# cts198859/deeprl_signal_control

Measured on NVIDIA H100. Metric: agent-env-steps/sec, higher is better.
Workload: dtype f32 (sim, LSTM cell, loss, optimizer) + bf16 tensor-core operands with f32 accumulation (learner GEMMs)

## Files before the change

deeprl_signal_control_b200/_lib.py:

```python
from __future__ import annotations

import ctypes as C
import os
import subprocess

_HERE = os.path.dirname(os.path.abspath(__file__))
CSRC = os.path.join(_HERE, "csrc")
LIB_PATH = os.environ.get("TSC_LIB", os.path.join(CSRC, "libtsc.so"))
_lib = None

SYMBOLS = ["tsc_last_error", "tsc_create", "tsc_destroy", "tsc_reset", "tsc_set_train_mode",
           "tsc_set_replica_coop_gamma", "tsc_observe", "tsc_step", "tsc_step_host", "tsc_step_host_range", "tsc_step_host_range_async", "tsc_set_record", "tsc_step_record", "tsc_get_trips", "tsc_get_counts", "tsc_get_traffic_stats",
           "tsc_dump_state", "tsc_info", "tsc_mean_live", "tsc_set_greedy_program", "tsc_greedy_actions",
           "tscl_create", "tscl_destroy", "tscl_fc_embed", "tscl_lstm_seq_fwd", "tscl_heads", "tscl_returns", "tscl_returns_g",
           "tscl_heads_loss", "tscl_lstm_seq_bwd", "tscl_fc_bwd", "tscl_fc_bwd_tc", "tscl_wgrad_tc", "tscl_clip_rmsprop",
           "tscl_pack_weights", "tscl_policy_step", "tscl_policy_step_v2", "tscl_policy_step_v2r", "tscl_policy_step_v2g", "tscl_unpack_store", "tscl_pack_wht", "tscl_lstm_seq_bwd_tc", "tscl_pack_wxt", "tscl_lstm_seq_bwd_tc_dx", "tscl_lstm_seq_bwd_tc_heads", "tscl_dx_tc", "tscl_dx_fc_bwd_tc", "tscl_host_transition", "tscl_device_transition", "tscl_device_transition_g","tscl_memcpy_async", "tscl_fc_hidden_fwd", "tscl_fc_hidden_bwd", "tscl_debug_policy_prof", "tscl_debug_bptt_prof",
           "tscl_policy_step_pi", "tscl_argmax_actions", "tscl_q_create", "tscl_q_destroy", "tscl_q_step",
           "tscl_q_explore", "tscl_q_sample", "tscl_q_td", "tscl_q_adam", "tscl_q_transition"]


def build_native(force: bool = False, verbose: bool = False) -> str:
    cmd = ["make", "-C", CSRC] + (["-B"] if force else [])
    out = subprocess.run(cmd, capture_output=True, text=True)
    if out.returncode != 0:
        raise RuntimeError("nvcc build of libtsc.so failed:\n" + out.stdout + out.stderr)
    if verbose:
        print(out.stdout + out.stderr)
    return LIB_PATH


def lib() -> C.CDLL:
    global _lib
    if _lib is None:
        if not os.path.exists(LIB_PATH):
            raise ImportError(
                "native library %s is missing: run `python -c 'import __graft_entry__ as g; g.build()'` "
                "(there is no CPU fallback)" % LIB_PATH)
        _lib = C.CDLL(LIB_PATH)
        _lib.tsc_last_error.restype = C.c_char_p
        for s in SYMBOLS:
            getattr(_lib, s)
    return _lib


def check(rc: int):
    if rc != 0:
        raise RuntimeError("libtsc: " + lib().tsc_last_error().decode())
```

deeprl_signal_control_b200/agents/learner.py:

```python
from __future__ import annotations

import ctypes as C
import os
import types
from typing import Optional, Sequence

import numpy as np
import torch

from .. import _lib
from .. import dist as _dist
from .layout import PolicyLayout


def _p(t):
    return None if t is None else C.c_void_p(t.data_ptr())


def check_population(seeds, seed, n_replicas, chunk, process_group):
    if seeds is None:
        return [int(seed)]
    seeds = [int(s) for s in seeds]
    if not seeds:
        raise ValueError("a population needs at least one seed")
# ... 127 lines not shown
        self.obs_hist = torch.zeros(T + 1, R, L.n_obs, **f32)
        self.act_hist = torch.zeros(T, R, A, dtype=torch.int32, device=self.dev)
        self.rew_hist = torch.zeros(T, R, A, **f32)
        self.val_hist = torch.zeros(T, R, A, **f32)
        self.Rs = torch.zeros(T, R, A, **f32); self.Adv = torch.zeros(T, R, A, **f32)
        self.done_pre = [0.0] * T
        self.done_post = [0.0] * T
        self.last_done = False
        self.t = 0
        self.n_forward = 0
        self._one = torch.zeros(1, **f32)
        self._upd_bufs = None
        self.kernel_launches = 0
        paths = self.paths
        self.use_tc, self.tc_v2 = paths.use_tc, paths.tc_v2
        mdim = () if self.K == 1 else (self.K,)
        self.Wp = torch.zeros(*mdim, U, ((L.dx + L.h) // 8) * 4 * L.h * 8 + 8 * L.dx * 8, dtype=torch.bfloat16,
                              device=self.dev)
        self.Wt = torch.zeros(*mdim, U, 32, L.h, 8, dtype=torch.bfloat16, device=self.dev)
        self.Wxt = torch.zeros(*mdim, U, 32, L.dx, 8, dtype=torch.bfloat16, device=self.dev)
        self.seeds_dev = torch.tensor(self.seeds, dtype=torch.int64, device=self.dev) if self.K > 1 else None
        differ = lambda *keys: any(len({h[k] for h in self.hp}) > 1 for k in keys)
        per = lambda key: torch.tensor([h[key] for h in self.hp], **f32)
        self.gamma_dev = per("gamma") if differ("gamma") else None
        self.rscale_differs = differ("reward_norm", "reward_clip")
        self.rnorm_dev, self.rclip_dev = (per("reward_norm"), per("reward_clip")) if self.rscale_differs else (None, None)
        self.dx_fused = False
        self.dx_fusable = paths.dx_fusable
        self.dx_own = paths.dx_own
        self.dx_fc_fused = paths.dx_fc_fused
        self.bwd_tc, self.fc_bwd_tc, self.wgrad_tc = paths.bwd_tc, paths.fc_bwd_tc, paths.wgrad_tc
        self.fused_heads = True
        self.heads_in_bptt = os.environ.get("TSC_BPTT_HEADS", "1") != "0"
        self._dz_all = None
        self.pack_weights()
        need = U * T * R * (L.dx + 4 * L.h + 2 * L.h) * 2
        if store_acts is None:
            free, _ = torch.cuda.mem_get_info(self.dev)
            store_acts = self.tc_v2 and need < 0.5 * free
        self.store_acts = bool(store_acts) and self.tc_v2 and (R % self.chunk == 0)
        if self.K > 1 and not self.store_acts:
            raise ValueError("a population back-propagates through the activation store, which does not fit: %.2f GB "
                             "for %d x %d replicas" % (need / 1e9, self.K, self.R_m))
        self.st_x = self.st_g = self.st_c = self.st_h = None
        if self.store_acts:
            bf = dict(dtype=torch.bfloat16, device=self.dev)
            nc, rc_ = R // self.chunk, self.chunk
            self.st_x = torch.zeros(nc, U, T, rc_, L.dx, **bf); self.st_g = torch.zeros(nc, U, T, rc_, 4 * L.h, **bf)
            self.st_c = torch.zeros(nc, U, T, rc_, L.h, **bf); self.st_h = torch.zeros(nc, U, T, rc_, L.h, **bf)
        self._acts_ok = [False] * T

    def close(self):
        if getattr(self, "_h", None) is not None:
            _lib.lib().tscl_destroy(self._h)
            self._h = None

    def __del__(self):
        try:
            self.close()
        except Exception:
            pass

    def member(self, k: int):
        if self.K == 1:
            return self
        return types.SimpleNamespace(lay=self.lay, _h=self._h, dev=self.dev, use_tc=self.use_tc, tc_v2=self.tc_v2,
# ... 188 lines not shown
        M = T * b["rc"]
        if (dh or not lean) and "dH" not in b:
            b["dH"] = torch.empty(U, M, L.h, **f32)
        if lean and dzb and "dZb" not in b:
            b["dZb"] = torch.empty(U, M, 4 * L.h, dtype=torch.bfloat16, device=self.dev)
        if lean and dxb and "dXb" not in b:
            b["dXb"] = torch.empty(U, M, L.dx, dtype=torch.bfloat16, device=self.dev)
        if not lean and "X" not in b:
            b.update(ZG=torch.empty(U, M, 4 * L.h, **f32), dX=torch.empty(U, M, L.dx, **f32),
                     X=torch.empty(U, M, L.dx, **f32), C=torch.empty(U, M, L.h, **f32), H=torch.empty(U, M, L.h, **f32),
                     Hp=torch.empty(U, M, L.h, **f32), dlog=torch.empty(U, M, L.max_na, **f32))
        return b

    def _dz_all_buf(self):
        if self._dz_all is None:
            L, nc = self.lay, self.R // self.chunk
            need = nc * L.U * self.T * self.chunk * 4 * L.h * 2
            free, _ = torch.cuda.mem_get_info(self.dev)
            if need >= 0.5 * free:
                return None
            if self._upd_bufs is not None:
                self._upd_bufs.pop("dZb", None)
            self._dz_all = torch.empty(nc, L.U, self.T * self.chunk, 4 * L.h, dtype=torch.bfloat16, device=self.dev)
        return self._dz_all

    def _bwd_heads(self, P, G, Wt, stats, r0, n_chunks, v_coef, beta, scale, dpre, dZb):
        ci, R, A = r0 // self.chunk, self.R, self.lay.A
        _lib.check(_lib.lib().tscl_lstm_seq_bwd_tc_heads(
            self._h, _p(Wt), _p(P), _p(self.st_g[ci]), _p(self.st_c[ci]), _p(self.st_h[ci]), _p(self.c_bw), _p(dpre),
            _p(self.act_hist[0, r0:]), _p(self.Rs[0, r0:]), _p(self.Adv[0, r0:]), C.c_int32(self.T),
            C.c_int64(self.chunk), C.c_int32(n_chunks), C.c_int64(R), C.c_int64(r0), C.c_int64(R * A), C.c_float(v_coef),
            C.c_float(beta), C.c_float(scale), _p(dZb), _p(stats), _p(G), self._st()))

    def backward(self, boot: Optional[torch.Tensor], lr: float, beta: float):
        assert self.t == self.T, "rollout buffer not full"
        L, R, T, U, A, lib = self.lay, self.R, self.T, self.lay.U, self.lay.A, _lib.lib()
        lrs, betas = self._per_member(lr, "lr"), self._per_member(beta, "beta")
        self._mm()
        st = self._st
        f32 = dict(dtype=torch.float32, device=self.dev)
        dpre = torch.tensor(self.done_pre, **f32)
        dpost = torch.tensor(self.done_post, **f32)
        if boot is None:
            self.boot.zero_()
        else:
            self.boot.copy_(boot)
        if self.gamma_dev is not None:
            _lib.check(lib.tscl_returns_g(self._h, _p(self.rew_hist), _p(self.val_hist), _p(self.boot), _p(dpost),
                                          _p(self.gamma_dev), C.c_int32(self.K), C.c_int32(T), C.c_int64(R), _p(self.Rs),
                                          _p(self.Adv), st()))
        else:
            _lib.check(lib.tscl_returns(self._h, _p(self.rew_hist), _p(self.val_hist), _p(self.boot), _p(dpost),
                                        C.c_float(self.gamma), C.c_int32(T), C.c_int64(R), _p(self.Rs), _p(self.Adv), st()))
        self.G.zero_()
        self.stats.zero_()
        scale = _dist.grad_scale(T, 1, self.total_replicas)
        use_store = self.store_acts and all(self._acts_ok)
        if self.K > 1 and not use_store:
            raise RuntimeError("a population update needs every step of the rollout in the activation store")
        n_obs = L.n_obs
        P, G, Wt, Wxt, stats = self.P, self.G, self.Wt, self.Wxt, self.stats
        k = 0
        lean = use_store and self.bwd_tc and self.fc_bwd_tc and self.wgrad_tc and self.fused_heads
        heads_bptt = lean and self.heads_in_bptt and not (self.dx_fused and self.dx_fusable)
        dz_all = self._dz_all_buf() if heads_bptt and self.K == 1 and R > self.chunk else None
        if dz_all is not None:
            self._bwd_heads(P, G, Wt, stats, 0, R // self.chunk, self.hp[0]["v_coef"], betas[0], scale, dpre, dz_all)
            self.kernel_launches += 1
        for r0 in range(0, R, self.chunk):
            if self.K > 1:
                k = r0 // self.R_m
                P, G, Wt, Wxt, stats = self.P[k], self.G[k], self.Wt[k], self.Wxt[k], self.stats[k]
            rc = min(self.chunk, R - r0)
            M = T * rc
            ci = r0 // self.chunk
            all_tc = lean
            fuse_dx = all_tc and self.dx_fused and self.dx_fusable
            fuse_fc = all_tc and not fuse_dx and self.dx_fc_fused
            b = self._bufs(rc, lean=all_tc, dxb=not fuse_fc, dh=not heads_bptt, dzb=dz_all is None)
            X = Cc = H = Hp = dlog = ZG = dX = dZb = dXb = dH = None
            bf16 = dict(dtype=torch.bfloat16, device=self.dev)
            if b["rc"] == rc:
                dH = b.get("dH")
                if all_tc:
                    dZb, dXb = (b["dZb"] if dz_all is None else dz_all[ci]), b.get("dXb")
                else:
                    ZG, dX, X, Cc, H, Hp, dlog = (b[k] for k in ("ZG", "dX", "X", "C", "H", "Hp", "dlog"))
            else:
                dH = torch.empty(U, M, L.h, **f32)
                if all_tc:
                    dZb = torch.empty(U, M, 4 * L.h, **bf16)
                    dXb = None if fuse_fc else torch.empty(U, M, L.dx, **bf16)
                else:
                    ZG, dX, X, Cc, H, Hp, dlog = (torch.empty(U, M, s_, **f32) for s_ in
                                                  (4 * L.h, L.dx, L.dx, L.h, L.h, L.h, L.max_na))
            obs0 = self.obs_hist[0, r0:]
            if all_tc:
                pass
            elif use_store:
                direct = self.bwd_tc
# ... 8 lines not shown
                torch.baddbmm(self.pv["bl"].unsqueeze(1), X, self.pv["wx"], out=ZG)
                _lib.check(lib.tscl_lstm_seq_fwd(self._h, _p(P), _p(ZG), _p(Cc), _p(H), _p(Hp), _p(self.c_bw),
                                                 _p(self.h_bw), None, None, _p(dpre), C.c_int32(T), C.c_int64(rc),
                                                 C.c_int64(R), C.c_int64(r0), st()))
            hb = _p(self.st_h[ci]) if use_store else None
            if heads_bptt:
                if dz_all is None:
                    self._bwd_heads(P, G, Wt, stats, r0, 1, self.hp[k]["v_coef"], betas[k], scale, dpre, dZb)
                    self.kernel_launches += 1
            else:
                _lib.check(lib.tscl_heads_loss(self._h, _p(P), None if all_tc else _p(H), _p(self.act_hist[0, r0:]),
                                               _p(self.Rs[0, r0:]), _p(self.Adv[0, r0:]), C.c_int64(M), C.c_int64(rc),
                                               C.c_int64(R * A), C.c_float(self.hp[k]["v_coef"]), C.c_float(betas[k]),
                                               C.c_float(scale),
                                               None if self.fused_heads else _p(dlog), _p(dH), _p(stats),
                                               hb if all_tc else None, _p(G) if self.fused_heads else None, st()))
                self.kernel_launches += 2
            if not self.fused_heads:
                self.gv["wo"].baddbmm_(H.transpose(1, 2), dlog)
                self.gv["bo"].add_(dlog.sum(dim=1))
            if heads_bptt:
                pass
            elif self.bwd_tc:
                gb = (_p(self.st_g[ci]), _p(self.st_c[ci])) if use_store else (None, None)
                _lib.check(lib.tscl_lstm_seq_bwd_tc_dx(self._h, _p(Wt), _p(ZG), _p(Cc), _p(dH), _p(self.c_bw),
                                                       _p(dpre), C.c_int32(T), C.c_int64(rc), C.c_int64(R), C.c_int64(r0),
                                                       *gb, _p(dZb), _p(Wxt) if fuse_dx else None,
                                                       _p(dXb) if fuse_dx else None, st()))
            else:
                _lib.check(lib.tscl_lstm_seq_bwd(self._h, _p(P), _p(ZG), _p(Cc), _p(dH), _p(self.c_bw), _p(dpre),
                                                 C.c_int32(T), C.c_int64(rc), C.c_int64(R), C.c_int64(r0), st()))
            dZ = ZG
            if self.wgrad_tc:
                if use_store:
                    _lib.check(lib.tscl_wgrad_tc(self._h, _p(dZ), _p(dZb), None, _p(self.st_x[ci]), None, _p(self.st_h[ci]),
                                                 _p(self.h_bw), _p(dpre), C.c_int32(T), C.c_int64(rc), C.c_int64(R),
                                                 C.c_int64(r0), _p(G), C.c_int32(0), st()))
                else:
                    _lib.check(lib.tscl_wgrad_tc(self._h, _p(dZ), None, _p(X), None, _p(Hp), None, None, None, C.c_int32(T),
                                                 C.c_int64(rc), C.c_int64(R), C.c_int64(r0), _p(G), C.c_int32(0), st()))
            else:
                self.gv["wx"].baddbmm_(X.transpose(1, 2), dZ)
                self.gv["wh"].baddbmm_(Hp.transpose(1, 2), dZ)
                self.gv["bl"].add_(dZ.sum(dim=1))
            if fuse_fc:
                _lib.check(lib.tscl_dx_fc_bwd_tc(self._h, _p(obs0), _p(self.st_x[ci]), _p(dZb), _p(Wxt), C.c_int64(M),
                                                 C.c_int64(rc), C.c_int64(R * n_obs), _p(G), st()))
            elif all_tc and not fuse_dx and self.dx_own:
                _lib.check(lib.tscl_dx_tc(self._h, _p(dZb), _p(Wxt), _p(dXb), C.c_int64(M), st()))
            elif all_tc and not fuse_dx:
                torch.bmm(dZb, self.wx_b.transpose(1, 2), out=dXb)
            elif not all_tc:
                torch.bmm(dZ, P[L.off_wx:L.off_wh].view(U, L.dx, 4 * L.h).transpose(1, 2), out=dX)
            if fuse_fc:
                pass
            elif self.fc_bwd_tc:
                xb = _p(self.st_x[ci]) if use_store else None
                _lib.check(lib.tscl_fc_bwd_tc(self._h, _p(obs0), None if all_tc else _p(X), xb, _p(dX), _p(dXb),
                                              C.c_int64(M), C.c_int64(rc), C.c_int64(R * n_obs), _p(G), C.c_int32(0),
                                              st()))
            else:
                _lib.check(lib.tscl_fc_bwd(self._h, _p(obs0), _p(X), _p(dX), C.c_int64(M), C.c_int64(rc),
                                           C.c_int64(R * n_obs), _p(G), st()))
            self.kernel_launches += 1 if fuse_fc else 2 if use_store else 3
        if self.pg is not None:
            _dist.allreduce_sum_(self.G, self.pg)
        for k in range(self.K):
# ... 13 lines not shown
```

deeprl_signal_control_b200/csrc/tsc_policy_tc.cu:

```cuda
#include <cuda.h>
#include <cstdlib>
#include <cuda_bf16.h>
#include <cuda_runtime.h>
#include <stdint.h>

#include <string>

#include "../../include/tsc_learn.h"

int tsc_set_error(const std::string& m);
#define PCK(call)                                                                  \
  do {                                                                             \
    cudaError_t e__ = (call);                                                      \
    if (e__ != cudaSuccess) return tsc_set_error(std::string(#call) + ": " + cudaGetErrorString(e__)); \
  } while (0)

struct DDimsTC {
  int A, n_obs, max_na, fw, ff, ft, h, dx;
  const int32_t *obs_off, *n_wave, *n_wait, *n_fp, *n_a;
  const int64_t *off_fcw_w, *off_fcw_b, *off_fcf_w, *off_fcf_b, *off_fct_w, *off_fct_b;
  int64_t off_wx, off_wh, off_bl, off_wo, off_bo, n_params;
  int kw, ones_slot;
};
const DDimsTC* tscl_dims_of(tscl_handle* h);
// ... 1654 lines not shown
        if (HEADS && t > 0) fetch_h(t - 1);
      }
      BR_MARK(3);
      wg_wait<0>();
      wg_frag_fence(acc);
      const bool need_dh = keep != 0.f && t > 0;
#pragma unroll
      for (int j = 0; j < 8; ++j)
#pragma unroll
        for (int e = 0; e < 4; ++e) dhc[j][e] = need_dh ? acc[4 * j + e] * keep : 0.f;
      BR_MARK(2);
    }
  }
  if (lead) asm volatile("cp.async.bulk.wait_group 0;" ::: "memory");
  if (HEADS) {
    if (cur_u >= 0) flush(cur_u);
    if (a.stats) {
#pragma unroll
      for (int o = 16; o; o >>= 1) {
        pl += __shfl_down_sync(0xffffffffu, pl, o);
        vl += __shfl_down_sync(0xffffffffu, vl, o);
        el += __shfl_down_sync(0xffffffffu, el, o);
      }
      if (lane == 0 && (pl != 0.f || vl != 0.f || el != 0.f)) {
        atomicAdd(&a.stats[0], pl * a.scale); atomicAdd(&a.stats[1], vl * a.scale); atomicAdd(&a.stats[2], el * a.scale);
      }
    }
  }
  if (PROF && lead)
    for (int i = 0; i < 4; ++i) atomicAdd(a.prof + i, (unsigned long long)bp[i]);
#undef BR_MARK
}

static bool make_tmap_3d(CUtensorMap* m, CUtensorMapDataType dt, int elem_bytes, const void* base, uint64_t planes,
                         uint64_t rows, uint64_t cols, uint32_t box_cols, uint32_t box_rows,
                         CUtensorMapSwizzle sw = CU_TENSOR_MAP_SWIZZLE_128B) {
  typedef CUresult (*encode_fn)(CUtensorMap*, CUtensorMapDataType, cuuint32_t, void*, const cuuint64_t*, const cuuint64_t*,
                                const cuuint32_t*, const cuuint32_t*, CUtensorMapInterleave, CUtensorMapSwizzle,
                                CUtensorMapL2promotion, CUtensorMapFloatOOBfill);
  static encode_fn fn = []() -> encode_fn {
    void* p = nullptr;
    cudaDriverEntryPointQueryResult q;
    if (cudaGetDriverEntryPoint("cuTensorMapEncodeTiled", &p, cudaEnableDefault, &q) != cudaSuccess || q != cudaDriverEntryPointSuccess)
      return nullptr;
    return (encode_fn)p;
  }();
  if (!fn || !base) return false;
  memset(m, 0, sizeof(*m));
  const cuuint64_t dims[3] = {cols, rows, planes};
  const cuuint64_t strides[2] = {cols * (uint64_t)elem_bytes, rows * cols * (uint64_t)elem_bytes};
  const cuuint32_t box[3] = {box_cols, box_rows, 1};
  const cuuint32_t es[3] = {1, 1, 1};
  return fn(m, dt, 3, const_cast<void*>(base), dims, strides, box, es, CU_TENSOR_MAP_INTERLEAVE_NONE, sw,
            CU_TENSOR_MAP_L2_PROMOTION_L2_128B, CU_TENSOR_MAP_FLOAT_OOB_FILL_NONE) == CUDA_SUCCESS;
}

__device__ __forceinline__ void cp_async16(uint32_t dst, const void* src) {
  asm volatile("cp.async.cg.shared.global [%0], [%1], 16;" ::"r"(dst), "l"(src) : "memory");
}

extern "C" int tscl_pack_wxt(tscl_handle* h, const float* params, void* wxt_bf16, void* stream) {
  if (!h || !params || !wxt_bf16) return tsc_set_error("tscl_pack_wxt: bad argument");
  PCK(cudaSetDevice(tscl_device_of(h)));
  const DDimsTC& d = *tscl_dims_of(h);
  pack_wxt_kernel<<<dim3(8, 2 * d.A), 256, 0, (cudaStream_t)stream>>>(d, params, (__nv_bfloat16*)wxt_bf16);
  PCK(cudaGetLastError());
  return 0;
}

extern "C" int tscl_pack_wht(tscl_handle* h, const float* params, void* wt_bf16, void* stream) {
  if (!h || !params || !wt_bf16) return tsc_set_error("tscl_pack_wht: bad argument");
  PCK(cudaSetDevice(tscl_device_of(h)));
  const DDimsTC& d = *tscl_dims_of(h);
  pack_wht_kernel<<<dim3(2, 2 * d.A), 256, 0, (cudaStream_t)stream>>>(d, params, (__nv_bfloat16*)wt_bf16);
  PCK(cudaGetLastError());
  return 0;
}

extern "C" int tscl_lstm_seq_bwd_tc(tscl_handle* h, const void* wt_bf16, float* ZG, const float* C, const float* dH,
// ... 665 lines not shown
    }
    *reinterpret_cast<uint4*>(sA + (size_t)(tid & 7) * WGA_SBO + arow * 16) = pv[4];
  };

  if (j0 < j1) { load_tile(); store_tile(0); }
  if (j0 + 1 < j1) load_tile();
  for (int64_t j = j0; j < j1; ++j) {
    const int u = (int)(j / tpu);
    const int s = (int)((j - j0) & 1);
    if (u != cur_u) {
      if (cur_u >= 0) flush(cur_u);
      cur_u = u; first = true;
    }
    asm volatile("fence.proxy.async.shared::cta;" ::: "memory");
    __syncthreads();
    const uint32_t aA = smem_u32(tc_smem + (size_t)s * WGA_STAGE), aZ = aA + WGA_A_CHUNKS * WGA_SBO;
    wg_fence();
    wg_mma_regs<64, 1, 1>(f, WGA_ROWS / 16, !first, [&](int ks, uint64_t& da, uint64_t& db) {
      da = make_desc(aA + ks * 256, lbo, sbo);
      db = make_desc(aZ + wq * 8 * WGA_SBO + ks * 256, lbo, sbo);
    });
    wg_commit();
    first = false;
    if (j + 1 < j1) {
      wg_wait<1>();
      __syncthreads();
      store_tile(s ^ 1);
      if (j + 2 < j1) load_tile();
    }
  }
  if (cur_u >= 0) flush(cur_u);
}

extern "C" int tscl_wgrad_tc(tscl_handle* h, const float* dZ, const void* dz_bf16, const float* X, const void* x_bf16,
                             const float* Hp, const void* h_bf16, const float* h0, const float* done, int32_t T, int64_t rc,
                             int64_t ld_state, int64_t r0, float* grads, int32_t variant, void* stream) {
  if (!h || (!dZ && !dz_bf16) || (!X && !x_bf16) || (!Hp && !h_bf16) || !grads || T <= 0 || rc <= 0)
    return tsc_set_error("tscl_wgrad_tc: bad argument");
  if (h_bf16 && (!h0 || !done)) return tsc_set_error("tscl_wgrad_tc: h_bf16 needs h0 and done");
  PCK(cudaSetDevice(tscl_device_of(h)));
  const DDimsTC& d = *tscl_dims_of(h);
  if ((d.dx % 8) != 0 || d.dx / 8 + 9 > WG_A_CHUNKS) return tsc_set_error("tscl_wgrad_tc: dx must be a multiple of 8, <= 240");
  const size_t smem = 2 * (size_t)WG_STAGE + 32;
  const size_t smem_async = (size_t)WGA_STAGES * WGA_STAGE + 4 * WGA_MAXT;
  static int attr_dev = -1;
  if (attr_dev != tscl_device_of(h)) {
    PCK(cudaFuncSetAttribute(wgrad_tc_kernel, cudaFuncAttributeMaxDynamicSharedMemorySize, (int)smem));
    PCK(cudaFuncSetAttribute(wgrad_tc_async_kernel, cudaFuncAttributeMaxDynamicSharedMemorySize, (int)smem_async));
    attr_dev = tscl_device_of(h);
  }
  int n_sm = 0;
  PCK(cudaDeviceGetAttribute(&n_sm, cudaDevAttrMultiProcessorCount, tscl_device_of(h)));
  const int64_t M = (int64_t)T * rc;
  const int64_t NT = ((M + FBT_ROWS - 1) / FBT_ROWS) * 4 * d.A;
  const int grid = (int)(NT < n_sm ? NT : n_sm);
  WGradTC a;
  a.acc = nullptr;
  a.dZ = dZ; a.dZb = (const __nv_bfloat16*)dz_bf16; a.X = X; a.Xb = (const __nv_bfloat16*)x_bf16; a.Hp = Hp; a.Hb = (const __nv_bfloat16*)h_bf16; a.h0 = h0;
  a.done = done; a.G = grads; a.M = M; a.rc = rc; a.ld_state = ld_state; a.r0 = r0; a.T = T; a.variant = variant;
  if (a.dZb && a.Xb && a.Hb && T <= WGA_MAXT) {
    const int64_t nt2 = ((M + WGA_ROWS - 1) / WGA_ROWS) * 2 * d.A;
    const int nsl = wga_slabs(d.dx);
    const int g2 = (int)(nt2 < n_sm / nsl ? nt2 : n_sm / nsl) * nsl;
    wgrad_tc_async_kernel<<<g2, FBT_THREADS, smem_async, (cudaStream_t)stream>>>(d, a);
  }
  else {
    a.acc = acc_tiles(h, stream);
    if (!a.acc) return tsc_set_error("accumulator tiles: cudaMalloc failed");
    wgrad_tc_kernel<<<grid, FBT_THREADS, smem, (cudaStream_t)stream>>>(d, a);
  }
  PCK(cudaGetLastError());
  return 0;
}

#define DXK_THREADS 384
#define DXK_STAGES 3
#define DXK_STAGE_BYTES 16384
struct DxTC {
  const __nv_bfloat16* dZb;
  const __nv_bfloat16* Wxt;
  __nv_bfloat16* dXb;
  int64_t M;
};
__device__ __forceinline__ uint64_t make_desc_sw128(uint32_t saddr) {
  return (uint64_t)((saddr >> 4) & 0x3FFFu) | (1ull << 16) | ((uint64_t)(1024 >> 4) << 32) | (1ull << 62);
}

template <int DXT>
__global__ void __launch_bounds__(DXK_THREADS, 1)
dx_tc_kernel(const DDimsTC d, const DxTC a) {
  constexpr int N64 = DXT / 64, R32 = (DXT % 64) >= 32, R16 = (DXT % 32) >= 16;
  const int tid = threadIdx.x, warp = tid >> 5, lane = tid & 31;
  const int dx = DXT, row_bytes = dx * 2, out_stride = row_bytes + 16;
  unsigned char* sStage = tc_smem;
  unsigned char* sB = sStage + DXK_STAGES * DXK_STAGE_BYTES;
  unsigned char* sOut = sB + (size_t)BW_KC * dx * 16;
  uint64_t* sBar = reinterpret_cast<uint64_t*>(sOut + (size_t)128 * out_stride);
  const uint32_t bar_full = smem_u32(sBar), bar_empty = bar_full + 24, bar_b = bar_full + 48;
  if (tid == 0) {
    for (int s = 0; s < DXK_STAGES; ++s) { mbar_init(bar_full + 8 * s, 128); mbar_init(bar_empty + 8 * s, 8); }
    mbar_init(bar_b, 1);
    asm volatile("fence.mbarrier_init.release.cluster;" ::: "memory");
  }
  __syncthreads();
// ... 486 lines not shown
```

include/tsc_learn.h:

```cpp
#ifndef TSC_LEARN_H_
#define TSC_LEARN_H_

#include <stdint.h>

#ifdef __cplusplus
extern "C" {
#endif

typedef struct tscl_dims {
  int32_t n_agents;
  int32_t n_obs;
  int32_t max_na;
  int32_t fw, ff, ft;
  int32_t h;
  int32_t dx;
  const int32_t* obs_off;
  const int32_t* n_wave;
  const int32_t* n_wait;
  const int32_t* n_fp;
  const int32_t* n_a;
  const int64_t* off_fcw_w;  const int64_t* off_fcw_b;
  const int64_t* off_fcf_w;  const int64_t* off_fcf_b;
  const int64_t* off_fct_w;  const int64_t* off_fct_b;
  int64_t off_wx;
// ... 17 lines not shown
                       float* dX, float* grads, void* stream);

int tscl_lstm_seq_fwd(tscl_handle* h, const float* params, float* ZG, float* C, float* H, float* Hprev,
                      const float* c0, const float* h0, float* c1, float* h1, const float* done, int32_t T,
                      int64_t Rc, int64_t ld_state, int64_t r0, void* stream);

int tscl_heads(tscl_handle* h, const float* params, const float* Hs, int64_t R, float* pi, float* val,
               int32_t* act, uint64_t seed, int64_t step, int64_t replica0, void* stream);

int tscl_returns(tscl_handle* h, const float* rew, const float* val, const float* boot, const float* done_post,
                 float gamma, int32_t T, int64_t R, float* Rs, float* Adv, void* stream);
int tscl_returns_g(tscl_handle* h, const float* rew, const float* val, const float* boot, const float* done_post,
                   const float* gamma, int32_t K, int32_t T, int64_t R, float* Rs, float* Adv, void* stream);

int tscl_heads_loss(tscl_handle* h, const float* params, const float* H, const int32_t* act, const float* Rs,
                    const float* Adv, int64_t M, int64_t Rc, int64_t stride_t, float v_coef, float beta,
                    float scale, float* dlog, float* dH, float* stats, const void* h_bf16, float* grads,
                    void* stream);

int tscl_lstm_seq_bwd(tscl_handle* h, const float* params, float* ZG, const float* C, const float* dH,
                      const float* c0, const float* done, int32_t T, int64_t Rc, int64_t ld_state, int64_t r0,
                      void* stream);

int tscl_fc_bwd(tscl_handle* h, const float* obs, const float* X, const float* dX, int64_t M,
                int64_t rows_per_t, int64_t stride_t, float* grads, void* stream);

int tscl_fc_bwd_tc(tscl_handle* h, const float* obs, const float* X, const void* x_bf16, const float* dX,
                   const void* dx_bf16, int64_t M, int64_t rows_per_t, int64_t stride_t, float* grads, int32_t variant,
                   void* stream);

int tscl_wgrad_tc(tscl_handle* h, const float* dZ, const void* dz_bf16, const float* X, const void* x_bf16,
                  const float* Hp, const void* h_bf16, const float* h0, const float* done, int32_t T, int64_t rc,
                  int64_t ld_state, int64_t r0, float* grads, int32_t variant, void* stream);

int tscl_pack_wht(tscl_handle* h, const float* params, void* wt_bf16, void* stream);
int tscl_lstm_seq_bwd_tc(tscl_handle* h, const void* wt_bf16, float* ZG, const float* C, const float* dH, const float* c0,
                         const float* done, int32_t T, int64_t Rc, int64_t ld_state, int64_t r0,
                         const void* gates_bf16, const void* c_bf16, void* dz_bf16, void* stream);
int tscl_pack_wxt(tscl_handle* h, const float* params, void* wxt_bf16, void* stream);
int tscl_lstm_seq_bwd_tc_dx(tscl_handle* h, const void* wt_bf16, float* ZG, const float* C, const float* dH, const float* c0,
                            const float* done, int32_t T, int64_t Rc, int64_t ld_state, int64_t r0,
                            const void* gates_bf16, const void* c_bf16, void* dz_bf16, const void* wxt_bf16, void* dx_bf16,
                            void* stream);
int tscl_lstm_seq_bwd_tc_heads(tscl_handle* h, const void* wt_bf16, const float* params, const void* gates_bf16,
                               const void* c_bf16, const void* h_bf16, const float* c0, const float* done,
                               const int32_t* act, const float* Rs, const float* Adv, int32_t T, int64_t Rc,
                               int32_t n_chunks, int64_t ld_state, int64_t r0, int64_t stride_t, float v_coef, float beta,
                               float scale, void* dz_bf16, float* stats, float* grads, void* stream);
int tscl_host_transition(tscl_handle* h, const float* obs_host, float* obs_dev, int64_t obs_floats, const float* rew_host,
                         float* rew_stage_dev, float* rew_hist_dev, int64_t rew_floats, float reward_norm, float reward_clip,
                         const float* grew_host, float* grew_stage_dev, float* rew_acc_dev, int64_t n, void* stream);
int tscl_device_transition(tscl_handle* h, const float* rew_dev, float* rew_hist_dev, int64_t rew_floats, float reward_norm,
                           float reward_clip, const float* grew_dev, float* rew_acc_dev, int64_t n, void* stream);
int tscl_device_transition_g(tscl_handle* h, const float* rew_dev, float* rew_hist_dev, int64_t rew_floats,
                             const float* reward_norm, const float* reward_clip, int32_t K, const float* grew_dev,
                             float* rew_acc_dev, int64_t n, void* stream);
int tscl_memcpy_async(tscl_handle* h, void* dst, const void* src, int64_t bytes, int32_t kind, void* stream);
int tscl_dx_tc(tscl_handle* h, const void* dz_bf16, const void* wxt_bf16, void* dx_bf16, int64_t M, void* stream);
int tscl_dx_fc_bwd_tc(tscl_handle* h, const float* obs, const void* x_bf16, const void* dz_bf16, const void* wxt_bf16,
                      int64_t M, int64_t rows_per_t, int64_t stride_t, float* grads, void* stream);

int tscl_unpack_store(tscl_handle* h, const void* st_x, const void* st_g, const void* st_c, const void* st_h, float* X,
                      float* ZG, float* C, float* H, float* Hp, const float* h0, const float* done, int32_t T,
                      int64_t rc, int64_t ld_state, int64_t r0, void* stream);

int tscl_debug_policy_prof(void* counters_dev);
// ... 72 lines not shown
```

Measured before the change: 31.99 million.

## Add TMA warp-specialized wgrad kernel and batch weight-gradient over all chunks

Adds a new weight-gradient kernel in which a producer warp loads dZ, X and H tiles through TMA into a 4-stage mbarrier ring, while consumer warps run wgmma and repartition registers with setmaxnreg. A new store entry point computes wgrad for all activation-store chunks in a single launch after the fused heads BPTT, instead of one launch per chunk. The goal is to overlap loads with tensor-core work and cut launch count. The cost is more complex code, extra atomics per fragment, and a fallback to the older per-chunk path when shape constraints fail.

```diff
diff --git a/deeprl_signal_control_b200/_lib.py b/deeprl_signal_control_b200/_lib.py
--- a/deeprl_signal_control_b200/_lib.py
+++ b/deeprl_signal_control_b200/_lib.py
@@ -13,7 +13,7 @@
            "tsc_set_replica_coop_gamma", "tsc_observe", "tsc_step", "tsc_step_host", "tsc_step_host_range", "tsc_step_host_range_async", "tsc_set_record", "tsc_step_record", "tsc_get_trips", "tsc_get_counts", "tsc_get_traffic_stats",
            "tsc_dump_state", "tsc_info", "tsc_mean_live", "tsc_set_greedy_program", "tsc_greedy_actions",
            "tscl_create", "tscl_destroy", "tscl_fc_embed", "tscl_lstm_seq_fwd", "tscl_heads", "tscl_returns", "tscl_returns_g",
-           "tscl_heads_loss", "tscl_lstm_seq_bwd", "tscl_fc_bwd", "tscl_fc_bwd_tc", "tscl_wgrad_tc", "tscl_clip_rmsprop",
+           "tscl_heads_loss", "tscl_lstm_seq_bwd", "tscl_fc_bwd", "tscl_fc_bwd_tc", "tscl_wgrad_tc", "tscl_wgrad_tc_store", "tscl_clip_rmsprop",
            "tscl_pack_weights", "tscl_policy_step", "tscl_policy_step_v2", "tscl_policy_step_v2r", "tscl_policy_step_v2g", "tscl_unpack_store", "tscl_pack_wht", "tscl_lstm_seq_bwd_tc", "tscl_pack_wxt", "tscl_lstm_seq_bwd_tc_dx", "tscl_lstm_seq_bwd_tc_heads", "tscl_dx_tc", "tscl_dx_fc_bwd_tc", "tscl_host_transition", "tscl_device_transition", "tscl_device_transition_g","tscl_memcpy_async", "tscl_fc_hidden_fwd", "tscl_fc_hidden_bwd", "tscl_debug_policy_prof", "tscl_debug_bptt_prof",
            "tscl_policy_step_pi", "tscl_argmax_actions", "tscl_q_create", "tscl_q_destroy", "tscl_q_step",
            "tscl_q_explore", "tscl_q_sample", "tscl_q_td", "tscl_q_adam", "tscl_q_transition"]
diff --git a/deeprl_signal_control_b200/agents/learner.py b/deeprl_signal_control_b200/agents/learner.py
--- a/deeprl_signal_control_b200/agents/learner.py
+++ b/deeprl_signal_control_b200/agents/learner.py
@@ -183,6 +183,7 @@
         self.bwd_tc, self.fc_bwd_tc, self.wgrad_tc = paths.bwd_tc, paths.fc_bwd_tc, paths.wgrad_tc
         self.fused_heads = True
         self.heads_in_bptt = os.environ.get("TSC_BPTT_HEADS", "1") != "0"
+        self.wgrad_tma = os.environ.get("TSC_WGRAD_TMA", "1") != "0"
         self._dz_all = None
         self.pack_weights()
         need = U * T * R * (L.dx + 4 * L.h + 2 * L.h) * 2
@@ -437,6 +438,13 @@
             C.c_int64(self.chunk), C.c_int32(n_chunks), C.c_int64(R), C.c_int64(r0), C.c_int64(R * A), C.c_float(v_coef),
             C.c_float(beta), C.c_float(scale), _p(dZb), _p(stats), _p(G), self._st()))
 
+    def _wgrad_store(self, G, r0, n_chunks, dpre, dZb):
+        ci = r0 // self.chunk
+        _lib.check(_lib.lib().tscl_wgrad_tc_store(
+            self._h, _p(dZb), _p(self.st_x[ci]), _p(self.st_h[ci]), _p(self.h_bw), _p(dpre), C.c_int32(self.T),
+            C.c_int64(self.chunk), C.c_int32(n_chunks), C.c_int64(self.R), C.c_int64(r0), _p(G),
+            C.c_int32(int(self.wgrad_tma)), self._st()))
+
     def backward(self, boot: Optional[torch.Tensor], lr: float, beta: float):
         assert self.t == self.T, "rollout buffer not full"
         L, R, T, U, A, lib = self.lay, self.R, self.T, self.lay.U, self.lay.A, _lib.lib()
@@ -471,6 +479,7 @@
         dz_all = self._dz_all_buf() if heads_bptt and self.K == 1 and R > self.chunk else None
         if dz_all is not None:
             self._bwd_heads(P, G, Wt, stats, 0, R // self.chunk, self.hp[0]["v_coef"], betas[0], scale, dpre, dz_all)
+            self._wgrad_store(G, 0, R // self.chunk, dpre, dz_all)
             self.kernel_launches += 1
         for r0 in range(0, R, self.chunk):
             if self.K > 1:
@@ -545,7 +554,11 @@
                                                  C.c_int32(T), C.c_int64(rc), C.c_int64(R), C.c_int64(r0), st()))
             dZ = ZG
             if self.wgrad_tc:
-                if use_store:
+                if dz_all is not None:
+                    pass
+                elif use_store and all_tc:
+                    self._wgrad_store(G, r0, 1, dpre, dZb)
+                elif use_store:
                     _lib.check(lib.tscl_wgrad_tc(self._h, _p(dZ), _p(dZb), None, _p(self.st_x[ci]), None, _p(self.st_h[ci]),
                                                  _p(self.h_bw), _p(dpre), C.c_int32(T), C.c_int64(rc), C.c_int64(R),
                                                  C.c_int64(r0), _p(G), C.c_int32(0), st()))
diff --git a/deeprl_signal_control_b200/csrc/tsc_policy_tc.cu b/deeprl_signal_control_b200/csrc/tsc_policy_tc.cu
--- a/deeprl_signal_control_b200/csrc/tsc_policy_tc.cu
+++ b/deeprl_signal_control_b200/csrc/tsc_policy_tc.cu
@@ -1710,19 +1710,24 @@
 #undef BR_MARK
 }
 
-static bool make_tmap_3d(CUtensorMap* m, CUtensorMapDataType dt, int elem_bytes, const void* base, uint64_t planes,
-                         uint64_t rows, uint64_t cols, uint32_t box_cols, uint32_t box_rows,
-                         CUtensorMapSwizzle sw = CU_TENSOR_MAP_SWIZZLE_128B) {
-  typedef CUresult (*encode_fn)(CUtensorMap*, CUtensorMapDataType, cuuint32_t, void*, const cuuint64_t*, const cuuint64_t*,
-                                const cuuint32_t*, const cuuint32_t*, CUtensorMapInterleave, CUtensorMapSwizzle,
-                                CUtensorMapL2promotion, CUtensorMapFloatOOBfill);
-  static encode_fn fn = []() -> encode_fn {
+typedef CUresult (*tmap_encode_fn)(CUtensorMap*, CUtensorMapDataType, cuuint32_t, void*, const cuuint64_t*, const cuuint64_t*,
+                                   const cuuint32_t*, const cuuint32_t*, CUtensorMapInterleave, CUtensorMapSwizzle,
+                                   CUtensorMapL2promotion, CUtensorMapFloatOOBfill);
+static tmap_encode_fn tmap_encoder() {
+  static tmap_encode_fn fn = []() -> tmap_encode_fn {
     void* p = nullptr;
     cudaDriverEntryPointQueryResult q;
     if (cudaGetDriverEntryPoint("cuTensorMapEncodeTiled", &p, cudaEnableDefault, &q) != cudaSuccess || q != cudaDriverEntryPointSuccess)
       return nullptr;
-    return (encode_fn)p;
+    return (tmap_encode_fn)p;
   }();
+  return fn;
+}
+
+static bool make_tmap_3d(CUtensorMap* m, CUtensorMapDataType dt, int elem_bytes, const void* base, uint64_t planes,
+                         uint64_t rows, uint64_t cols, uint32_t box_cols, uint32_t box_rows,
+                         CUtensorMapSwizzle sw = CU_TENSOR_MAP_SWIZZLE_128B) {
+  const tmap_encode_fn fn = tmap_encoder();
   if (!fn || !base) return false;
   memset(m, 0, sizeof(*m));
   const cuuint64_t dims[3] = {cols, rows, planes};
@@ -2454,15 +2459,234 @@
   if (cur_u >= 0) flush(cur_u);
 }
 
-extern "C" int tscl_wgrad_tc(tscl_handle* h, const float* dZ, const void* dz_bf16, const float* X, const void* x_bf16,
-                             const float* Hp, const void* h_bf16, const float* h0, const float* done, int32_t T, int64_t rc,
-                             int64_t ld_state, int64_t r0, float* grads, int32_t variant, void* stream) {
+#define WGT_STAGES 4
+#define WGT_Z_BYTES (32 * 1024)
+#define WGT_STAGE (WGT_Z_BYTES + 16 * 1024)
+#define WGT_THREADS (FBT_THREADS + 128)
+#define WGT_PROD_REGS 24
+#define WGT_CONS_REGS 112
+static_assert(128 * WGT_PROD_REGS + FBT_THREADS * WGT_CONS_REGS <= WGT_THREADS * 96, "setmaxnreg split exceeds the CTA's registers");
+#define WGT_SMEM (WGT_STAGES * WGT_STAGE + 4 * WGA_MAXT + 16 * WGT_STAGES)
+struct WGradTMA {
+  const float* h0;
+  const float* done;
+  float* G;
+  int64_t M, rc, ld_state, r0;
+  int T, n_chunks, variant;
+};
+__device__ __forceinline__ uint64_t make_desc_mn_sw128(uint32_t saddr) {
+  return (uint64_t)((saddr >> 4) & 0x3FFFu) | ((uint64_t)(8192 >> 4) << 16) | ((uint64_t)(1024 >> 4) << 32) | (1ull << 62);
+}
+__device__ __forceinline__ uint64_t make_desc_mn_sw64(uint32_t saddr, bool swap) {
+  const uint64_t lbo = swap ? 512 : 4096, sbo = swap ? 4096 : 512;
+  return (uint64_t)((saddr >> 4) & 0x3FFFu) | ((lbo >> 4) << 16) | ((sbo >> 4) << 32) | (2ull << 62);
+}
+__device__ __forceinline__ int sw64_off(int r, int e) { return r * 64 + ((e ^ ((r >> 1) & 3)) << 4); }
+
+__global__ void __launch_bounds__(WGT_THREADS, 1)
+wgrad_tc_tma_kernel(const DDimsTC d, const WGradTMA a, const __grid_constant__ CUtensorMap mapZ,
+                    const __grid_constant__ CUtensorMap mapX, const __grid_constant__ CUtensorMap mapH) {
+  const int tid = threadIdx.x, warp = tid >> 5, lane = tid & 31, wq = warp >> 2;
+  float* sDone = reinterpret_cast<float*>(tc_smem + WGT_STAGES * WGT_STAGE);
+  const uint32_t full0 = smem_u32(sDone + WGA_MAXT), empty0 = full0 + 8 * WGT_STAGES;
+  const int dx = d.dx, ng = dx >> 3, ncta = (wga_slabs(dx) + 1) / 2;
+  const int ngrp = gridDim.x / ncta, pb = blockIdx.x / ncta, sl0 = 2 * (blockIdx.x - pb * ncta);
+  const int64_t tpu = (a.M + WGA_ROWS - 1) / WGA_ROWS;
+  const int64_t NT = tpu * 2 * d.A;
+  const int64_t j0 = NT * pb / ngrp, j1 = NT * (pb + 1) / ngrp;
+  for (int i = tid; i < WGT_STAGES * 16 * WGA_ROWS; i += WGT_THREADS) {
+    const int s = i / (16 * WGA_ROWS), k = (i / WGA_ROWS) & 15, row = i % WGA_ROWS, cg = sl0 * 8 + k;
+    if (cg >= ng + 8)
+      *reinterpret_cast<uint4*>(tc_smem + (size_t)s * WGT_STAGE + WGT_Z_BYTES + (k >> 2) * 4096 + sw64_off(row, k & 3)) =
+          make_uint4(cg == ng + 8 ? 0x3f80u : 0u, 0, 0, 0);
+  }
+  for (int i = tid; i < a.T; i += WGT_THREADS) sDone[i] = a.done[i];
+  if (tid == 0) {
+    for (int s = 0; s < WGT_STAGES; ++s) { mbar_init(full0 + 8 * s, 1); mbar_init(empty0 + 8 * s, 16); }
+    asm volatile("fence.mbarrier_init.release.cluster;" ::: "memory");
+  }
+  asm volatile("fence.proxy.async.shared::cta;" ::: "memory");
+  __syncthreads();
+  const int u0 = (int)(j0 / tpu);
+  const int64_t tile0 = j0 - (int64_t)u0 * tpu;
+
+  if (warp >= 16) {
+    asm volatile("setmaxnreg.dec.sync.aligned.u32 %0;" ::"n"(WGT_PROD_REGS));
+    if (warp == 16 && lane == 0) {
+      uint32_t bytes = WGT_Z_BYTES;
+      for (int q = 0; q < 4; ++q) if (sl0 * 8 + 4 * q < ng + 8) bytes += 4096;
+      int64_t k = 0;
+      for (int c = 0; c < a.n_chunks; ++c) {
+        int u = u0;
+        int64_t tile = tile0;
+        for (int64_t j = j0; j < j1; ++j, ++k) {
+          const int s = (int)(k % WGT_STAGES);
+          if (k >= WGT_STAGES) mbar_wait(empty0 + 8 * s, (uint32_t)((k / WGT_STAGES - 1) & 1));
+          const uint32_t full = full0 + 8 * s, dst = smem_u32(tc_smem + (size_t)s * WGT_STAGE);
+          const int m0 = (int)(tile * WGA_ROWS);
+          mbar_expect_tx(full, bytes);
+          for (int q = 0; q < 4; ++q) tma_load_3d(dst + 8192 * q, &mapZ, 64 * q, m0, c * 2 * d.A + u, full);
+          for (int q = 0; q < 4; ++q) {
+            const int cg = sl0 * 8 + 4 * q;
+            if (cg < ng) tma_load_3d(dst + WGT_Z_BYTES + 4096 * q, &mapX, 8 * cg, m0, c * 2 * d.A + u, full);
+            else if (cg < ng + 8)
+              tma_load_3d(dst + WGT_Z_BYTES + 4096 * q, &mapH, 8 * (cg - ng), m0 - (int)a.rc, c * 2 * d.A + u, full);
+          }
+          if (++tile == tpu) { tile = 0; ++u; }
+        }
+      }
+    }
+    return;
+  }
+
+  asm volatile("setmaxnreg.inc.sync.aligned.u32 %0;" ::"n"(WGT_CONS_REGS));
+  const bool has_hp = sl0 * 8 < ng + 8 && sl0 * 8 + 16 > ng;
+  float f0[32], f1[32];
+  auto flush_frag = [&](const float (&f)[32], int uu, int o) {
+#pragma unroll
+    for (int hh = 0; hh < 2; ++hh) {
+      const int ci = (sl0 + o) * 64 + (warp & 3) * 16 + (lane >> 2) + 8 * hh;
+      float* dst = nullptr;
+      if (ci < dx) dst = a.G + d.off_wx + ((int64_t)uu * dx + ci) * TC_N;
+      else if (ci < dx + TC_H) dst = a.G + d.off_wh + ((int64_t)uu * TC_H + (ci - dx)) * TC_N;
+      else if (ci == dx + TC_H) dst = a.G + d.off_bl + (int64_t)uu * TC_N;
+      if (dst) {
+        dst += wq * 64 + 2 * (lane & 3);
+#pragma unroll
+        for (int i = 0; i < 8; ++i) { atomicAdd(dst + 8 * i, f[4 * i + 2 * hh]); atomicAdd(dst + 8 * i + 1, f[4 * i + 2 * hh + 1]); }
+      }
+    }
+  };
+  auto flush = [&](int uu) {
+    wg_wait<0>();
+    wg_frag_fence(f0);
+    wg_frag_fence(f1);
+    flush_frag(f0, uu, 0);
+    flush_frag(f1, uu, 1);
+  };
+  int64_t k = 0;
+  int prev_s = -1;
+  for (int c = 0; c < a.n_chunks; ++c) {
+    int u = u0, cur_u = -1;
+    int64_t tile = tile0;
+    int64_t it_t = tile * WGA_ROWS / a.rc, it_rem = tile * WGA_ROWS - it_t * a.rc;
+    bool first = true;
+    for (int64_t j = j0; j < j1; ++j, ++k) {
+      const int s = (int)(k % WGT_STAGES);
+      if (u != cur_u) {
+        if (cur_u >= 0) flush(cur_u);
+        cur_u = u; first = true;
+      }
+      unsigned char* sA = tc_smem + (size_t)s * WGT_STAGE + WGT_Z_BYTES;
+      const int64_t m0 = tile * WGA_ROWS;
+      const int rows_valid = (a.M - m0) < WGA_ROWS ? (int)(a.M - m0) : WGA_ROWS;
+      mbar_wait(full0 + 8 * s, (uint32_t)((k / WGT_STAGES) & 1));
+      if (has_hp) {
+        bool fix = it_t == 0 || sDone[it_t] != 0.f;
+        for (int64_t t = it_t, r = it_rem + rows_valid - 1; r >= a.rc;) { r -= a.rc; ++t; fix |= sDone[t] != 0.f; }
+        if (fix) {
+          wg_wait<0>();
+          const int row = tid >> 3;
+#pragma unroll
+          for (int o = 0; o < 2; ++o) {
+            const int kk = 8 * o + (tid & 7), hc = sl0 * 8 + kk - ng;
+            if (hc >= 0 && hc < 8 && row < rows_valid) {
+              int64_t t = it_t, rem = it_rem + row;
+              while (rem >= a.rc) { rem -= a.rc; ++t; }
+              uint4* dst = reinterpret_cast<uint4*>(sA + (kk >> 2) * 4096 + sw64_off(row, kk & 3));
+              if (sDone[t] != 0.f) *dst = make_uint4(0, 0, 0, 0);
+              else if (t == 0) {
+                const float4* hp = reinterpret_cast<const float4*>(
+                    a.h0 + ((int64_t)u * a.ld_state + a.r0 + (int64_t)c * a.rc + rem) * TC_H + hc * 8);
+                const float4 p = __ldg(hp), qv = __ldg(hp + 1);
+                __align__(16) __nv_bfloat16 tt[8] = {__float2bfloat16_rn(p.x), __float2bfloat16_rn(p.y), __float2bfloat16_rn(p.z),
+                                                     __float2bfloat16_rn(p.w), __float2bfloat16_rn(qv.x), __float2bfloat16_rn(qv.y),
+                                                     __float2bfloat16_rn(qv.z), __float2bfloat16_rn(qv.w)};
+                *dst = *reinterpret_cast<const uint4*>(tt);
+              }
+            }
+          }
+          asm volatile("fence.proxy.async.shared::cta;" ::: "memory");
+          asm volatile("bar.sync 1, 512;" ::: "memory");
+        }
+      }
+      const uint32_t aZ = smem_u32(tc_smem + (size_t)s * WGT_STAGE) + wq * 8192, aA = smem_u32(sA);
+      wg_fence();
+      wg_mma_regs<64, 1, 1>(f0, WGA_ROWS / 16, !first, [&](int ks, uint64_t& da, uint64_t& db) {
+        da = make_desc_mn_sw64(aA + ks * 1024, a.variant != 0);
+        db = make_desc_mn_sw128(aZ + ks * 2048);
+      });
+      wg_mma_regs<64, 1, 1>(f1, WGA_ROWS / 16, !first, [&](int ks, uint64_t& da, uint64_t& db) {
+        da = make_desc_mn_sw64(aA + 8192 + ks * 1024, a.variant != 0);
+        db = make_desc_mn_sw128(aZ + ks * 2048);
+      });
+      wg_commit();
+      first = false;
+      wg_wait<1>();
+      if (prev_s >= 0) {
+        __syncwarp();
+        if (lane == 0) mbar_arrive(empty0 + 8 * prev_s);
+      }
+      prev_s = s;
+      it_rem += WGA_ROWS;
+      while (it_rem >= a.rc) { it_rem -= a.rc; ++it_t; }
+      if (++tile == tpu) { tile = 0; it_t = 0; it_rem = 0; ++u; }
+    }
+    if (cur_u >= 0) flush(cur_u);
+  }
+}
+
+static int wgrad_tma_launch(tscl_handle* h, const DDimsTC& d, const void* dz_bf16, const void* x_bf16, const void* h_bf16,
+                            const float* h0, const float* done, int32_t T, int64_t rc, int32_t n_chunks, int64_t ld_state,
+                            int64_t r0, float* grads, int32_t variant, void* stream) {
+  const int64_t M = (int64_t)T * rc;
+  const uint64_t U = (uint64_t)2 * d.A;
+  CUtensorMap mZ, mX, mH;
+  if (!(make_tmap_3d(&mZ, CU_TENSOR_MAP_DATA_TYPE_BFLOAT16, 2, dz_bf16, n_chunks * U, M, TC_N, 64, WGA_ROWS) &&
+        make_tmap_3d(&mX, CU_TENSOR_MAP_DATA_TYPE_BFLOAT16, 2, x_bf16, n_chunks * U, M, d.dx, 32, WGA_ROWS,
+                     CU_TENSOR_MAP_SWIZZLE_64B) &&
+        make_tmap_3d(&mH, CU_TENSOR_MAP_DATA_TYPE_BFLOAT16, 2, h_bf16, n_chunks * U, M, TC_H, 32, WGA_ROWS,
+                     CU_TENSOR_MAP_SWIZZLE_64B)))
+    return 1;
+  static int attr_dev = -1;
+  if (attr_dev != tscl_device_of(h)) {
+    PCK(cudaFuncSetAttribute(wgrad_tc_tma_kernel, cudaFuncAttributeMaxDynamicSharedMemorySize, WGT_SMEM));
+    attr_dev = tscl_device_of(h);
+  }
+  int n_sm = 0;
+  PCK(cudaDeviceGetAttribute(&n_sm, cudaDevAttrMultiProcessorCount, tscl_device_of(h)));
+  const int64_t nt = ((M + WGA_ROWS - 1) / WGA_ROWS) * 2 * d.A;
+  const int ncta = (wga_slabs(d.dx) + 1) / 2;
+  const int grid = (int)(nt < n_sm / ncta ? nt : n_sm / ncta) * ncta;
+  WGradTMA a;
+  a.h0 = h0; a.done = done; a.G = grads; a.M = M; a.rc = rc; a.ld_state = ld_state; a.r0 = r0; a.T = T;
+  a.n_chunks = n_chunks; a.variant = variant;
+  wgrad_tc_tma_kernel<<<grid, WGT_THREADS, WGT_SMEM, (cudaStream_t)stream>>>(d, a, mZ, mX, mH);
+  PCK(cudaGetLastError());
+  return 0;
+}
+static bool wgrad_tma_fits(const DDimsTC& d, int32_t T, int64_t rc) {
+  return d.dx % 32 == 0 && T <= WGA_MAXT && (int64_t)T * rc + rc <= 0x7fffffff;
+}
+
+static bool wgrad_tma_default() {
+  const char* e = getenv("TSC_WGRAD_TMA");
+  return !(e && atoi(e) == 0);
+}
+
+static int wgrad_tc_chunk(tscl_handle* h, const float* dZ, const void* dz_bf16, const float* X, const void* x_bf16,
+                          const float* Hp, const void* h_bf16, const float* h0, const float* done, int32_t T, int64_t rc,
+                          int64_t ld_state, int64_t r0, float* grads, int32_t variant, bool tma, void* stream) {
   if (!h || (!dZ && !dz_bf16) || (!X && !x_bf16) || (!Hp && !h_bf16) || !grads || T <= 0 || rc <= 0)
     return tsc_set_error("tscl_wgrad_tc: bad argument");
   if (h_bf16 && (!h0 || !done)) return tsc_set_error("tscl_wgrad_tc: h_bf16 needs h0 and done");
   PCK(cudaSetDevice(tscl_device_of(h)));
   const DDimsTC& d = *tscl_dims_of(h);
   if ((d.dx % 8) != 0 || d.dx / 8 + 9 > WG_A_CHUNKS) return tsc_set_error("tscl_wgrad_tc: dx must be a multiple of 8, <= 240");
+  if (tma && dz_bf16 && x_bf16 && h_bf16 && wgrad_tma_fits(d, T, rc)) {
+    const int r = wgrad_tma_launch(h, d, dz_bf16, x_bf16, h_bf16, h0, done, T, rc, 1, ld_state, r0, grads, variant, stream);
+    if (r != 1) return r;
+  }
   const size_t smem = 2 * (size_t)WG_STAGE + 32;
   const size_t smem_async = (size_t)WGA_STAGES * WGA_STAGE + 4 * WGA_MAXT;
   static int attr_dev = -1;
@@ -2492,6 +2716,35 @@
     wgrad_tc_kernel<<<grid, FBT_THREADS, smem, (cudaStream_t)stream>>>(d, a);
   }
   PCK(cudaGetLastError());
+  return 0;
+}
+
+extern "C" int tscl_wgrad_tc(tscl_handle* h, const float* dZ, const void* dz_bf16, const float* X, const void* x_bf16,
+                             const float* Hp, const void* h_bf16, const float* h0, const float* done, int32_t T, int64_t rc,
+                             int64_t ld_state, int64_t r0, float* grads, int32_t variant, void* stream) {
+  return wgrad_tc_chunk(h, dZ, dz_bf16, X, x_bf16, Hp, h_bf16, h0, done, T, rc, ld_state, r0, grads, variant,
+                        wgrad_tma_default(), stream);
+}
+
+extern "C" int tscl_wgrad_tc_store(tscl_handle* h, const void* dz_bf16, const void* x_bf16, const void* h_bf16,
+                                   const float* h0, const float* done, int32_t T, int64_t rc, int32_t n_chunks,
+                                   int64_t ld_state, int64_t r0, float* grads, int32_t tma, void* stream) {
+  if (!h || !dz_bf16 || !x_bf16 || !h_bf16 || !h0 || !done || !grads || T <= 0 || rc <= 0 || n_chunks <= 0)
+    return tsc_set_error("tscl_wgrad_tc_store: bad argument");
+  PCK(cudaSetDevice(tscl_device_of(h)));
+  const DDimsTC& d = *tscl_dims_of(h);
+  if (tma && n_chunks > 1 && wgrad_tma_fits(d, T, rc)) {
+    const int r = wgrad_tma_launch(h, d, dz_bf16, x_bf16, h_bf16, h0, done, T, rc, n_chunks, ld_state, r0, grads, 0, stream);
+    if (r != 1) return r;
+  }
+  const int64_t U = 2 * d.A, M = (int64_t)T * rc;
+  for (int c = 0; c < n_chunks; ++c) {
+    const int r = wgrad_tc_chunk(h, nullptr, (const __nv_bfloat16*)dz_bf16 + c * U * M * TC_N, nullptr,
+                                 (const __nv_bfloat16*)x_bf16 + c * U * M * d.dx, nullptr,
+                                 (const __nv_bfloat16*)h_bf16 + c * U * M * TC_H, h0, done, T, rc, ld_state, r0 + c * rc,
+                                 grads, 0, tma != 0, stream);
+    if (r) return r;
+  }
   return 0;
 }
 
diff --git a/include/tsc_learn.h b/include/tsc_learn.h
--- a/include/tsc_learn.h
+++ b/include/tsc_learn.h
@@ -73,6 +73,9 @@
 int tscl_wgrad_tc(tscl_handle* h, const float* dZ, const void* dz_bf16, const float* X, const void* x_bf16,
                   const float* Hp, const void* h_bf16, const float* h0, const float* done, int32_t T, int64_t rc,
                   int64_t ld_state, int64_t r0, float* grads, int32_t variant, void* stream);
+int tscl_wgrad_tc_store(tscl_handle* h, const void* dz_bf16, const void* x_bf16, const void* h_bf16, const float* h0,
+                        const float* done, int32_t T, int64_t rc, int32_t n_chunks, int64_t ld_state, int64_t r0,
+                        float* grads, int32_t tma, void* stream);
 
 int tscl_pack_wht(tscl_handle* h, const float* params, void* wt_bf16, void* stream);
 int tscl_lstm_seq_bwd_tc(tscl_handle* h, const void* wt_bf16, float* ZG, const float* C, const float* dH, const float* c0,
```

Result: no change. 32.22 million (median of 6 runs) (+0.7%).
